# ricklisz/AnatoMask

Hardware: AMD Instinct MI355X
Metric: pretrain volumes/sec @128^3 patch mask=0.6 (higher is better)
Workload: dtype bf16; 1 GPU; STUNet-B AnatoMask step, 128^3 patch, mask_ratio 0.6, bf16 storage/MFMA + fp32 master; per_gpu_batch=16, global_batch=16, parallelism=dp1, step=teacher fwd + sampler + student fwd + loss + bwd + clip + AdamW + EMA

## Files before the change

### anatomask_amd/csrc/stream_ops.hip

```cpp
#include <mutex>
#include <type_traits>
#include "common.h"
#include "../../include/anatomask_hip.h"

namespace {

constexpr int NREP = 8;

struct Geo {
  int B, D, H, W, C;
  int vpw;
  unsigned mW, mH, mD;
  MaskView mask;
  __device__ __forceinline__ bool active(long v) const {
    if (!mask.m) return true;
    const unsigned u = (unsigned)v;
    const unsigned t1 = __umulhi(u, mW); const int w = u - t1 * W;
    const unsigned t2 = __umulhi(t1, mH); const int h = t1 - t2 * H;
    const unsigned b = __umulhi(t2, mD); const int d = t2 - b * D;
    return mask.active((int)b, d, h, w);
  }
  __device__ __forceinline__ void decode(long v, int& b, int& d, int& h, int& w) const {
    const unsigned u = (unsigned)v;
    const unsigned t1 = __umulhi(u, mW); w = u - t1 * W;
// ... 1242 lines not shown
    const double b1 = wc * S0, b2 = rs * wc * S1;
    const float gr = fin.gamma[c] * fin.rstd[c];
    fin.k0w[c] = gr * fin.w[c]; fin.k1[c] = gr * (float)(b1 / fin.n); fin.k2[c] = gr * (float)(b2 / fin.n);
    fin.dgamma[c] += (float)b2;
    fin.dbeta[c] += (float)b1;
    fin.dw[c] += (float)((double)fin.scale[c] * S1 + (double)fin.beta[c] * S0);
  }
  if (threadIdx.x == 0) atomicExch(fin.ticket, 0u);
}

template <typename T>
__global__ __launch_bounds__(256) void proj_norm_bwd_apply_kernel(const T* __restrict__ x, const float* __restrict__ drec, long nvox, int C,
                                                                  int vpw, const float* __restrict__ mean, const float* __restrict__ rstd,
                                                                  const float* __restrict__ k0w, const float* __restrict__ k1,
                                                                  const float* __restrict__ k2, T* __restrict__ dx) {
  constexpr int EPC = TT<T>::EPC;
  Walk<T> wk(C);
  if (!wk.live) return;
  float mu[EPC], c0[EPC], c1[EPC], c2[EPC];
#pragma unroll
  for (int i = 0; i < EPC; ++i) {
    const int c = wk.cl * EPC + i;
    mu[i] = mean[c]; c0[i] = k0w[c]; c1[i] = k1[c]; c2[i] = k2[c] * rstd[c];
  }
  const long v0 = (long)blockIdx.x * vpw, v1 = min(v0 + (long)vpw, nvox);
  for (long v = v0 + wk.vl; v < v1; v += wk.vpp) {
    const float d = drec[v];
    const size_t off = (size_t)v * C + wk.cl * EPC;
    float f[EPC], r[EPC];
    chunk_to_f<T>(*(const u32x4*)(x + off), f);
#pragma unroll
    for (int i = 0; i < EPC; ++i) r[i] = c0[i] * d - c1[i] - c2[i] * (f[i] - mu[i]);
    *(u32x4*)(dx + off) = f_to_chunk<T>(r);
  }
}

template <typename T>
__global__ __launch_bounds__(256) void proj_bwd_kernel(const T* __restrict__ x, const float* __restrict__ drec, long nvox, int C, int vpw,
                                                       const float* __restrict__ w, T* __restrict__ dx, float* __restrict__ dw,
                                                       float* __restrict__ db, float* __restrict__ det_ws) {
  constexpr int EPC = TT<T>::EPC;
  __shared__ float red[256 * 8];
  __shared__ float redb[4];
  Walk<T> wk(C);
  float sw[EPC], wv[EPC], sb = 0.f;
#pragma unroll
  for (int i = 0; i < EPC; ++i) { sw[i] = 0.f; wv[i] = wk.live ? w[wk.cl * EPC + i] : 0.f; }
  const long v0 = (long)blockIdx.x * vpw, v1 = min(v0 + (long)vpw, nvox);
  if (wk.live)
    for (long v = v0 + wk.vl; v < v1; v += wk.vpp) {
      const float d = drec[v];
      const size_t off = (size_t)v * C + wk.cl * EPC;
      float f[EPC], o[EPC];
      chunk_to_f<T>(*(const u32x4*)(x + off), f);
#pragma unroll
      for (int i = 0; i < EPC; ++i) { sw[i] += d * f[i]; o[i] = d * wv[i]; }
      *(u32x4*)(dx + off) = f_to_chunk<T>(o);
      if (wk.cl == 0) sb += d;
    }
#pragma unroll
  for (int i = 0; i < EPC; ++i) red[threadIdx.x * 8 + i] = sw[i];
  sb = warp_sum(sb);
  if ((threadIdx.x & 63) == 0) redb[threadIdx.x >> 6] = sb;
  __syncthreads();
  if (threadIdx.x < wk.cpv) {
    float a1[EPC];
// ... 597 lines not shown
  hipStream_t st = (hipStream_t)stream;
  const int nb = (int)((nvox + 255) / 256);
  am_by_dtype(dtype, [&](auto t) {
    using T = typename decltype(t)::type;
    AM_LAUNCH(proj_fwd_kernel<T>, dim3(nb), dim3(256), 0, st, (const T*)x, nvox, C, w, b, pre_scale, pre_shift, rec);
  });
  AM_CHECK_LAUNCH();
  return 0;
}

int am_proj_norm_bwd(int dtype, const void* x, const float* drec, long nvox, int C, const float* w, const float* gamma, const float* beta,
                     const float* mean, const float* rstd, const float* scale, double* workspace, float* coef, void* dx,
                     float* dgamma_accum, float* dbeta_accum, float* dw_accum, float* db_accum, void* stream) {
  if (!am_row_ok(dtype, C, F32_MAX_C_256)) return -1;
  if (!x || !drec || !w || !gamma || !beta || !mean || !rstd || !scale || !workspace || !coef || !dx || !dgamma_accum || !dbeta_accum ||
      !dw_accum || !db_accum || nvox <= 0) return -1;
  hipStream_t st = (hipStream_t)stream;
  ProjNormFin fin{(unsigned*)(workspace + (size_t)NREP * (C + 1)), (double)nvox, gamma, beta, rstd, scale, w,
                  coef, coef + C, coef + 2 * C, dgamma_accum, dbeta_accum, dw_accum, db_accum};
  const int vr = pick_vpw(nvox, C, dtype, true), va = pick_vpw(nvox, C, dtype, false);
  am_by_dtype(dtype, [&](auto t) {
    using T = typename decltype(t)::type;
    AM_LAUNCH(proj_norm_bwd_reduce_kernel<T>, dim3(nblk(nvox, vr)), dim3(256), 0, st, (const T*)x, drec, nvox, C, vr, mean, workspace, fin);
  });
  AM_CHECK_LAUNCH();
  am_by_dtype(dtype, [&](auto t) {
    using T = typename decltype(t)::type;
    AM_LAUNCH(proj_norm_bwd_apply_kernel<T>, dim3(nblk(nvox, va)), dim3(256), 0, st, (const T*)x, drec, nvox, C, va, mean, rstd, coef, coef + C, coef + 2 * C, (T*)dx);
  });
  AM_CHECK_LAUNCH();
  return 0;
}

int am_proj_bwd(int dtype, const void* x, const float* drec, long nvox, int C, const float* w, void* dx, float* dw_accum,
                float* db_accum, float* det_workspace, long det_workspace_floats, void* stream) {
  if (!am_row_ok(dtype, C, F32_MAX_C_256)) return -1;
  hipStream_t st = (hipStream_t)stream;
  const int vpw = pick_vpw(nvox, C, dtype, true);
  const int nb = nblk(nvox, vpw);
  if (det_workspace && det_workspace_floats < (long)nb * (C + 1)) return -6;
  am_by_dtype(dtype, [&](auto t) {
    using T = typename decltype(t)::type;
    AM_LAUNCH(proj_bwd_kernel<T>, dim3(nb), dim3(256), 0, st, (const T*)x, drec, nvox, C, vpw, w, (T*)dx, dw_accum, db_accum, det_workspace);
  });
  AM_CHECK_LAUNCH();
  if (det_workspace) {
    AM_LAUNCH(rows_fold_kernel, dim3((C + 1 + 255) / 256), dim3(256), 0, st, det_workspace, nb, C + 1, C, dw_accum, db_accum);
    AM_CHECK_LAUNCH();
  }
  return 0;
}

int am_partials_reduce(const float* partials, int rows, int C, double* sums, float* sum_accum, void* stream) {
  hipStream_t st = (hipStream_t)stream;
  if ((256 % C == 0 || C % 256 == 0) && rows >= 64) {
    const int rstep = C <= 256 ? 256 / C : 1;
    int nb = rows / (rstep * 16); nb = nb < 1 ? 1 : (nb > 256 ? 256 : nb);
    const int rpb = ((rows + nb - 1) / nb + rstep - 1) / rstep * rstep;
    nb = (rows + rpb - 1) / rpb;
    if (sums) AM_HIP(hipMemsetAsync(sums, 0, sizeof(double) * 2 * C, st));
    AM_LAUNCH(partials_reduce2_kernel, dim3(nb), dim3(256), 0, st, partials, rows, C, rpb, sums, sum_accum);
    AM_CHECK_LAUNCH();
    return 0;
  }
  AM_LAUNCH(partials_reduce_kernel, dim3(C), dim3(256), 0, st, partials, rows, C, sums, sum_accum);
  AM_CHECK_LAUNCH();
// ... 78 lines not shown
```

### anatomask_amd/engine.py

```python
from __future__ import annotations

from dataclasses import dataclass, field
from typing import Dict, List, Optional, Sequence, Tuple

import torch

from . import ops
from .ops import ACT_LRELU, ACT_NONE, ACT_RELU6, CONV_DGRAD, CONV_FWD, CONVT_DGRAD, CONVT_FWD, MaskInfo, NormStats

ENC = "sparse_encoder.sp_cnn.conv_blocks_context"
DEC = "dense_decoder.dec"


@dataclass
class Spec:
    dims: Sequence[int]
    depth: Sequence[int]
    width: int
    input_size: Tuple[int, int, int]
    in_ch: int = 1
    out_ch: int = 1
    downsample: int = 16
    n_stage: int = 5
    sync_bn: bool = False
    dec_inorm: bool = False
    enc_chs: List[int] = field(init=False)
    dec_chs: List[int] = field(init=False)
    fmap: Tuple[int, int, int] = field(init=False)

    def __post_init__(self):
        assert self.in_ch == 1 and self.out_ch == 1, "the AnatoMask recipe is single-channel CT (P/pretrain_AntoMask.py:188)"
        assert all(s % self.downsample == 0 for s in self.input_size)
        self.enc_chs = list(self.dims[:5])
        n = 4
        self.dec_chs = [self.width // 2 ** i for i in range(n + 1)]
        self.fmap = tuple(s // self.downsample for s in self.input_size)
        assert all(c % 8 == 0 for c in self.enc_chs + self.dec_chs), "channel counts must be multiples of 8"

    def stage_spatial(self, s: int) -> Tuple[int, int, int]:
        return tuple(v >> s for v in self.input_size)


class Tape:

    def __init__(self):
        self.enc: List[dict] = []
        self.dens: List[dict] = []
        self.dec: List[dict] = []
        self.last: Optional[torch.Tensor] = None
        self.counts: Dict[int, torch.Tensor] = {}
        self.recompute = False
        self.enc_in: List[Optional[torch.Tensor]] = []


def _counts(mask: MaskInfo, levels: Sequence[int]) -> Dict[int, object]:
    if mask.n_active is not None:
        return {bs: float(mask.n_active) * float((1 << bs) ** 3) for bs in levels}
    out = {}
    buf = torch.empty(len(levels), device=mask.t.device, dtype=torch.float64)
    for i, bs in enumerate(levels):
        ops.mask_count(mask, (1 << bs) ** 3, buf[i:i + 1])
        out[bs] = buf[i:i + 1]
    return out


def _set_count(st: NormStats, cnt):
    if isinstance(cnt, float):
        st.count_host, st.count_ptr = cnt, None
    else:
        st.count_ptr = cnt


def _sparse_norm(x, mask, bs, counts, gamma, beta, eps, part=None) -> NormStats:
    st = NormStats(x.shape[-1], x.device)
    _set_count(st, counts[bs])
    if part is not None:
        part.finalize(st, gamma, beta, eps)
        return st
    ops.chan_stats(x, mask, bs, st)
    ops.norm_finalize(st, gamma, beta, eps)
    return st


def _sync_world(sync: bool) -> int:
    import torch.distributed as dist
# ... 203 lines not shown
        if tape is not None and recompute:
            tape.enc_in.append(x)
        for b in range(spec.depth[s]):
            x, rec_ = _enc_block(W, pk, inp, mask, counts, sp, s, b, x, keep=tape is not None)
            if tape is not None and not recompute:
                tape.enc.append(rec_)
        feats.append(x)
    return feats


def densify_forward(spec: Spec, W, pk: PackCache, feats, mask: MaskInfo, counts, tape: Optional[Tape] = None) -> List[torch.Tensor]:
    n_dec = len(spec.dec_chs) - 1
    to_dec = []
    for i in range(n_dec):
        f = feats[4 - i]
        st = _sparse_norm(f, mask, i, counts, W[f"densify_norms.{i}.weight"], W[f"densify_norms.{i}.bias"], 1e-6)
        d = ops.norm_apply(f, st, ACT_NONE, mask, i, fill=W[f"mask_tokens.{i}"].view(-1))
        pw = f"densify_projs.{i}.weight"
        if pw in W:
            k = W[pw].shape[-1]
            pr = ops.conv3d(CONV_FWD, d, pk.get(W, pw, False, False), W[f"densify_projs.{i}.bias"], tuple(d.shape[1:4]), k, 1)
        else:
            pr = d
        to_dec.append(pr)
        if tape is not None:
            tape.dens.append({"i": i, "f": f, "st": st, "d": d, "k": W[pw].shape[-1] if pw in W else 0})
    return to_dec


HEAD_STENCIL = True


def decoder_forward(spec: Spec, W, pk: PackCache, to_dec, train: bool, tape: Optional[Tape] = None, recompute: bool = False,
                    needed_patches: Optional[MaskInfo] = None, fuse_eval: Optional[bool] = None, l2_of: Optional[tuple] = None) -> torch.Tensor:
    n_dec = len(spec.dec_chs) - 1
    if fuse_eval is None:
        fuse_eval = tape is None
    x = to_dec[0]
    head = bool(train and FUSED_HEAD and _sync_world(spec.sync_bn) <= 1 and not spec.dec_inorm)
    st_head = None
    for i in range(n_dec):
        nxt = to_dec[i + 1] if i + 1 < n_dec else None
        last = i == n_dec - 1
        o, rec_ = _dec_block(W, pk, i, x, nxt, train, fuse_eval=fuse_eval,
                             out_skip=needed_patches if (last and tape is None and not train) else None, sync=spec.sync_bn,
                             head=head and last, inorm=spec.dec_inorm,
                             stencil_tail=bool(HEAD_STENCIL and last and tape is None and not train and fuse_eval and not spec.dec_inorm))
        if rec_ is not None and rec_.get("stencil"):
            q = f"{DEC}.{i}"
            weff, beff = ops.head_fold(W[f"{q}.conv.3.weight"], rec_["st2"].scale, rec_["st2"].shift, W["dense_decoder.proj.weight"].view(-1),
                                       W["dense_decoder.proj.bias"])
            B_, D_, H_, W_ = o.shape[:4]
            patches = needed_patches
            if patches is None:
                patches = MaskInfo(torch.ones(B_, D_ // 16, H_ // 16, W_ // 16, device=o.device, dtype=torch.uint8), n_active=B_ * (D_ // 16) * (H_ // 16) * (W_ // 16))
            if l2_of is not None:
                ops.head_stencil(o, weff, beff, patches, inp=l2_of[0], l2=l2_of[1])
                return None
            rec = torch.empty(B_, D_, H_, W_, device=o.device, dtype=torch.float32)
            ops.head_stencil(o, weff, beff, patches, rec=rec)
            return rec
        if head and last:
            st_head = rec_["st2"]
        if tape is not None:
            tape.dec.append({"q": rec_["q"], "xin": x, "nxt": nxt, "head": head and last} if recompute else rec_)
        x = o
    rec = ops.proj_fwd(x, W["dense_decoder.proj.weight"].view(-1), W["dense_decoder.proj.bias"], pre=st_head)
    if tape is not None:
        tape.last = x
    return rec


def forward(spec: Spec, W: Dict[str, torch.Tensor], pk: PackCache, inp: torch.Tensor, mask: MaskInfo, train: bool,
            tape: Optional[Tape] = None, want_feats: bool = False, encoder_only: bool = False, recompute: bool = False,
            want_to_dec0: bool = False, needed_patches: Optional[MaskInfo] = None, l2_out: Optional[torch.Tensor] = None):
    counts = _counts(mask, range(5))
    if tape is not None:
        tape.counts = counts
        tape.recompute = recompute
    feats = encoder_forward(spec, W, pk, inp, mask, counts, tape, recompute)
    if encoder_only:
        return feats
    to_dec = densify_forward(spec, W, pk, feats, mask, counts, tape)
    rec = decoder_forward(spec, W, pk, to_dec, train, tape, recompute, needed_patches, l2_of=(inp, l2_out) if l2_out is not None else None)
    if want_to_dec0:
        return rec, to_dec[0]
    return (rec, feats) if want_feats else rec


FUSED_HEAD = True
_SIDE: Dict[int, "torch.cuda.Stream"] = {}
_SIDE_KEEP: Dict[int, List[torch.Tensor]] = {}
_USE_SIDE = True


def _dev_index(dev) -> int:
    return dev.index if dev.index is not None else torch.cuda.current_device()


def _side_stream(dev) -> "torch.cuda.Stream":
    i = _dev_index(dev)
    if i not in _SIDE:
        _SIDE[i] = torch.cuda.Stream(device=dev)
    return _SIDE[i]


def _on_side(dev, tensors, fn):
    if not _USE_SIDE:
        return fn()
    s2 = _side_stream(dev)
    ev = torch.cuda.Event()
    ev.record()
    s2.wait_event(ev)
    _SIDE_KEEP.setdefault(_dev_index(dev), []).extend(tensors)
    with torch.cuda.stream(s2):
        fn()


def _join_side(dev):
    i = _dev_index(dev)
    if _USE_SIDE and i in _SIDE:
        ev = torch.cuda.Event()
        ev.record(_SIDE[i])
        torch.cuda.current_stream(dev).wait_event(ev)
    _SIDE_KEEP.pop(i, None)


def _wgrad_into(pk: PackCache, G, name, mode, x, dy, k, stride, transposed=False, **masks):
    def run():
        dwp = ops.conv3d_wgrad(mode, x, dy, k, stride, f32_split=pk.f32_split, deterministic=pk.deterministic, **masks)
        ops.unpack_grad(dwp, G[name], transposed, accumulate=True)
    _on_side(x.device, (x, dy), run)


def _dec_block_backward(W, G, pk: PackCache, t: dict, g: Optional[torch.Tensor], drec: Optional[torch.Tensor], bias_sum_into: Optional[torch.Tensor]):
    q = t["q"]
    if t.get("inorm"):
        so = tuple(t["r"].shape[1:4])
        dc2 = _instance_norm_backward(g, t["c2"], t["st2"], ACT_NONE)
        dr = ops.conv3d(CONV_DGRAD, dc2, pk.get(W, f"{q}.conv.3.weight", False, True), None, so, 3, 1)
        _wgrad_into(pk, G, f"{q}.conv.3.weight", CONV_FWD, t["r"], dc2, 3, 1)
        dc1 = _instance_norm_backward(dr, t["c1"], t["st1"], ACT_RELU6)
    elif t.get("head"):
        dc2 = ops.proj_norm_bwd(t["c2"], t["st2"], drec, W["dense_decoder.proj.weight"].view(-1), W[f"{q}.conv.4.weight"],
                                W[f"{q}.conv.4.bias"], G[f"{q}.conv.4.weight"], G[f"{q}.conv.4.bias"],
                                G["dense_decoder.proj.weight"].view(-1), G["dense_decoder.proj.bias"])
    else:
        dc2 = ops.norm_backward(g, None, t["c2"], t["st2"], W[f"{q}.conv.4.weight"], ACT_NONE, None, 0,
                                G[f"{q}.conv.4.weight"], G[f"{q}.conv.4.bias"])
    if not t.get("inorm"):
        so = tuple(t["r"].shape[1:4])
        fuse = ops.FUSED_NORM_BWD_REDUCE and dc2.dtype == torch.bfloat16 and t["st1"].sync_world <= 1 and dc2.shape[-1] >= 128
        dr = ops.conv3d(CONV_DGRAD, dc2, pk.get(W, f"{q}.conv.3.weight", False, True), None, so, 3, 1,
                        norm_bwd=(t["c1"], t["st1"], ACT_RELU6) if fuse else None)
        dr, red1 = dr if fuse else (dr, None)
        _wgrad_into(pk, G, f"{q}.conv.3.weight", CONV_FWD, t["r"], dc2, 3, 1)
        dc1 = ops.norm_backward(dr, None, t["c1"], t["st1"], W[f"{q}.conv.1.weight"], ACT_RELU6, None, 0,
                                G[f"{q}.conv.1.weight"], G[f"{q}.conv.1.bias"], reduced=red1)
    du, ptu = ops.conv3d(CONV_DGRAD, dc1, pk.get(W, f"{q}.conv.0.weight", False, True), None, so, 3, 1, want_partials=True, partials_sum_only=True)
    ptu.finalize(None, sum_accum=G[f"{q}.up_sample.bias"])
    _wgrad_into(pk, G, f"{q}.conv.0.weight", CONV_FWD, t["u"], dc1, 3, 1)
    si = tuple(t["xin"].shape[1:4])
    gin = ops.conv3d(CONVT_DGRAD, du, pk.get(W, f"{q}.up_sample.weight", True, True), None, si, 4, 2, want_partials=bias_sum_into is not None)
    if bias_sum_into is not None:
        gin, ptg = gin
        ptg.finalize(None, sum_accum=bias_sum_into)
    _wgrad_into(pk, G, f"{q}.up_sample.weight", CONVT_FWD, t["xin"], du, 4, 2, transposed=True)
    return gin


def decoder_backward(spec: Spec, W, G, pk: PackCache, tape: Tape, drec: torch.Tensor, after_group=None) -> List[Optional[torch.Tensor]]:
    n_dec = len(spec.dec_chs) - 1
    fused_head = bool(tape.dec[n_dec - 1].get("head"))
    g = None
    if not fused_head:
        g = ops.proj_bwd(tape.last, drec, W["dense_decoder.proj.weight"].view(-1), G["dense_decoder.proj.weight"].view(-1),
                         G["dense_decoder.proj.bias"], deterministic=pk.deterministic)
        if after_group:
            after_group("proj")
    dproj: List[Optional[torch.Tensor]] = [None] * n_dec
    for i in reversed(range(n_dec)):
        t = tape.dec[i]
        if tape.recompute:
            _, t = _dec_block(W, pk, i, t["xin"], t["nxt"], True, update_running=False, sync=spec.sync_bn, head=bool(t.get("head")),
                              inorm=spec.dec_inorm)
            tape.dec[i] = None
        if i + 1 < n_dec:
            dproj[i + 1] = g
        need_sum = i > 0 and f"densify_projs.{i}.bias" in G
        g = _dec_block_backward(W, G, pk, t, g, drec, G[f"densify_projs.{i}.bias"] if need_sum else None)
        if t.get("head") and after_group:
            after_group("proj")
        if after_group:
            after_group(f"dec{i}")
    dproj[0] = g
    return dproj


def densify_backward(spec: Spec, W, G, pk: PackCache, mask: MaskInfo, tape: Tape, dproj) -> List[Optional[torch.Tensor]]:
    n_dec = len(spec.dec_chs) - 1
    dfeat: List[Optional[torch.Tensor]] = [None] * spec.n_stage
    for i in range(n_dec):
        t = tape.dens[i]
        dp = dproj[i]
        if t["k"]:
            pw = f"densify_projs.{i}.weight"
            dd = ops.conv3d(CONV_DGRAD, dp, pk.get(W, pw, False, True), None, tuple(dp.shape[1:4]), t["k"], 1)
            _wgrad_into(pk, G, pw, CONV_FWD, t["d"], dp, t["k"], 1)
            if i == 0:
                ops.chan_sum(dp, None, 0, G[f"densify_projs.{i}.bias"])
        else:
            dd = dp
        dfeat[4 - i] = ops.norm_backward(dd, None, t["f"], t["st"], W[f"densify_norms.{i}.weight"], ACT_NONE, mask, i,
                                         G[f"densify_norms.{i}.weight"], G[f"densify_norms.{i}.bias"],
                                         dtoken=G[f"mask_tokens.{i}"].view(-1), fill=True)
    return dfeat


def _enc_block_backward(W, G, pk: PackCache, inp: torch.Tensor, mask: MaskInfo, t: dict, gout: torch.Tensor, base: Optional[torch.Tensor],
                        free_saved: bool = False) -> Optional[torch.Tensor]:
    p, s = t["p"], t["s"]
    bs = 4 - s
    y2, a1, y1, out, x = t["y2"], t["a1"], t["y1"], t["out"], t["x"]
# ... 127 lines not shown
```

### anatomask_amd/ops.py

```python
from __future__ import annotations

from typing import Optional, Tuple

import torch

from . import hip
from .hip import ACT_LRELU, ACT_NONE, ACT_RELU6, CONV_DGRAD, CONV_FWD, CONVT_DGRAD, CONVT_FWD


def _dt(t: torch.Tensor) -> int:
    if t.dtype == torch.float32:
        return hip.DT_F32
    if t.dtype == torch.bfloat16:
        return hip.DT_BF16
    raise TypeError(f"unsupported dtype {t.dtype}")


DEFAULT_F32_SPLIT = False


def _dtc(t: torch.Tensor, f32_split: bool) -> int:
    return hip.DT_F32S if (t.dtype == torch.float32 and f32_split) else _dt(t)


# ... 466 lines not shown
    B, D, H, W, Cc = x.shape
    mp, fd, fh, fw = _mk(mask)
    hip.lib().chan_sum(_dt(x), x.data_ptr(), B, D, H, W, Cc, mp, bshift, fd, fh, fw, out_accum.data_ptr(), _stream())


def add(a: torch.Tensor, b: torch.Tensor, out: Optional[torch.Tensor] = None) -> torch.Tensor:
    if out is None:
        out = torch.empty_like(a)
    hip.lib().add(_dt(a), a.data_ptr(), b.data_ptr(), out.data_ptr(), a.numel(), _stream())
    return out


def proj_fwd(x: torch.Tensor, w: torch.Tensor, b: torch.Tensor, pre: Optional["NormStats"] = None) -> torch.Tensor:
    B, D, H, W, Cc = x.shape
    rec = torch.empty(B, D, H, W, device=x.device, dtype=torch.float32)
    hip.lib().proj_fwd(_dt(x), x.data_ptr(), B * D * H * W, Cc, w.data_ptr(), b.data_ptr(), _p(pre.scale) if pre else None,
                       _p(pre.shift) if pre else None, rec.data_ptr(), _stream())
    return rec


def proj_norm_bwd(x: torch.Tensor, st: "NormStats", drec: torch.Tensor, w: torch.Tensor, gamma: torch.Tensor, beta: torch.Tensor,
                  dgamma: torch.Tensor, dbeta: torch.Tensor, dw_accum: torch.Tensor, db_accum: torch.Tensor) -> torch.Tensor:
    B, D, H, W, Cc = x.shape
    assert st.sync_world <= 1
    dx = torch.empty_like(x)
    ws_b, _ = _bwd_workspaces(x.device, Cc)
    coef = torch.empty(3, Cc, device=x.device, dtype=torch.float32)
    hip.lib().proj_norm_bwd(_dt(x), x.data_ptr(), drec.data_ptr(), B * D * H * W, Cc, w.data_ptr(), gamma.data_ptr(), beta.data_ptr(),
                            st.mean.data_ptr(), st.rstd.data_ptr(), st.scale.data_ptr(), ws_b.data_ptr(), coef.data_ptr(), dx.data_ptr(),
                            dgamma.data_ptr(), dbeta.data_ptr(), dw_accum.data_ptr(), db_accum.data_ptr(), _stream())
    return dx


def proj_bwd(x: torch.Tensor, drec: torch.Tensor, w: torch.Tensor, dw_accum: torch.Tensor, db_accum: torch.Tensor,
             deterministic: Optional[bool] = None) -> torch.Tensor:
    B, D, H, W, Cc = x.shape
    dx = torch.empty_like(x)
    ws = _det_workspace(x.device, 4096 * (Cc + 1) // 8) if _det(deterministic) else None
    hip.lib().proj_bwd(_dt(x), x.data_ptr(), drec.data_ptr(), B * D * H * W, Cc, w.data_ptr(), dx.data_ptr(), dw_accum.data_ptr(),
                       db_accum.data_ptr(), _p(ws), ws.numel() if ws is not None else 0, _stream())
    return dx


def head_stencil_supported(x: torch.Tensor) -> bool:
    B, D, H, W, C = x.shape
    ok = hip.lib()._lib.am_head_stencil_supported(_dt(x), C) == 1
    return bool(ok and D % 16 == 0 and H % 16 == 0 and W % 16 == 0 and max(B, D // 16, H // 16, W // 16) <= 255)


def head_fold(w2: torch.Tensor, scale: torch.Tensor, shift: torch.Tensor, wproj: torch.Tensor, bproj: torch.Tensor):
    cmid, cin = w2.shape[0], w2.shape[1]
    assert tuple(w2.shape[2:]) == (3, 3, 3) and w2.is_contiguous() and wproj.numel() == cmid
    weff = torch.empty(27, cin, device=w2.device, dtype=torch.float32)
    beff = torch.empty(1, device=w2.device, dtype=torch.float32)
    hip.lib().head_fold(w2.data_ptr(), cmid, cin, scale.data_ptr(), shift.data_ptr(), wproj.data_ptr(), bproj.data_ptr(), weff.data_ptr(),
                        beff.data_ptr(), _stream())
    return weff, beff


def head_stencil(r: torch.Tensor, weff: torch.Tensor, beff: torch.Tensor, patches: MaskInfo, rec: Optional[torch.Tensor] = None,
                 inp: Optional[torch.Tensor] = None, l2: Optional[torch.Tensor] = None):
    B, D, H, W, C = r.shape
    lst, n = patches.active_list()
    assert lst is not None and (patches.fd, patches.fh, patches.fw) == (D // 16, H // 16, W // 16) and r.is_contiguous()
    assert rec is None or (rec.dtype == torch.float32 and tuple(rec.shape) == (B, D, H, W) and rec.is_contiguous())
    assert l2 is None or (inp is not None and l2.dtype == torch.float32 and l2.numel() == B * patches.fd * patches.fh * patches.fw)
# ... 133 lines not shown
```

### anatomask_amd/trainer.py

```python
from __future__ import annotations

from typing import Dict, Optional

import torch
import torch.distributed as dist

from . import engine, ops
from .modules import ModelEma, SparK, ema_decay_for_epoch


class _Range:
    __slots__ = ("on",)

    def __init__(self, on: bool, name: str):
        self.on = on
        if on:
            torch.cuda.nvtx.range_push(name)

    def __enter__(self):
        return self

    def __exit__(self, *exc):
        if self.on:
            torch.cuda.nvtx.range_pop()
# ... 213 lines not shown
    def step(self, inp_bchwd: torch.Tensor, epoch: int = 0, mask1: Optional[torch.Tensor] = None,
             keys: Optional[torch.Tensor] = None, lr: Optional[float] = None, ema_decay: Optional[float] = None):
        m, t = self.model, self.teacher.ema
        spec = m.spec
        x = inp_bchwd[:, 0].float().contiguous()
        B = x.shape[0]
        L = spec.fmap[0] * spec.fmap[1] * spec.fmap[2]
        dev = x.device
        if mask1 is None:
            k1 = torch.rand(B, L, device=dev, generator=self.gen)
            m1 = ops.mask_sampler(torch.zeros(B, L, device=dev), k1, m.len_keep, 0)
        else:
            m1 = mask1.reshape(B, L).to(device=dev, dtype=torch.uint8).contiguous()
        mi1 = ops.MaskInfo(m1.view(B, *spec.fmap), n_active=B * m.len_keep if mask1 is None else None)
        tr_ = self.trace_ranges
        if self.self_distill:
            with _Range(tr_, "anatomask.teacher_forward"):
                need = ops.MaskInfo((1 - m1).view(B, *spec.fmap), n_active=B * (L - m.len_keep) if mask1 is None else None) if spec.input_size[0] // spec.fmap[0] == 16 else None
                recon = torch.zeros(B, L, device=dev) if need is not None else None
                rec1 = engine.forward(spec, t._W, t._pack, x, mi1, train=False, needed_patches=need, l2_out=recon)
                if rec1 is not None:
                    recon, _, _, _ = ops.patch_loss_fwd(x, rec1, mi1, normalized=False, want_loss=False)
                del rec1
            with _Range(tr_, "anatomask.mask_sampler"):
                ll = m.len_loss_for(L, m.len_keep, epoch, self.total_epochs - 1, self.guide)
                if keys is None:
                    keys = torch.rand(B, L, device=dev, generator=self.gen)
                mk = ops.mask_sampler(recon, keys.to(dev).float().contiguous(), m.len_keep, ll)
                mi = ops.MaskInfo(mk.view(B, *spec.fmap), n_active=B * m.len_keep)
        else:
            recon, mk, mi = None, m1, mi1
        self._snap_b.copy_(m._bflat); self._snap_i.copy_(m._iflat)
        tape = engine.Tape()
        with _Range(tr_, "anatomask.student_forward"):
            rec = engine.forward(spec, m._W, m._pack, x, mi, train=True, tape=tape, recompute=m.recompute)
            l2m, pm, pr, info = ops.patch_loss_fwd(x, rec, mi, normalized=True)
            drec = ops.patch_loss_bwd(x, rec, mi, pm, pr, info, None)
        with _Range(tr_, "anatomask.backward"):
            m._gflat.zero_()
            if self.distributed and not self._capturing:
                self._exchange_begin()
            engine.backward(spec, m._W, m._G, m._pack, x, mi, tape, drec, self._after_group if self.distributed else None, join_before_hook=False)
            del tape
        with _Range(tr_, "anatomask.exchange_wait"):
            self._finish_exchange()
        rng_opt = _Range(tr_, "anatomask.optimizer_ema")
        n = m._live_end
        decay = self.teacher.decay if ema_decay is None else ema_decay
        ops.sumsq(m._gflat[:n], self.sumsq)
        dyn = None
        if self._capturing:
            dyn = self._dyn_dev
        else:
            self.step_count += 1
        ops.adamw_ema(m._flat, m._gflat, self.m, self.v, t._flat if self.self_distill else None, n, self.lr if lr is None else lr,
                      self.betas, self.eps, self.wd, max(self.step_count, 1), self.sumsq, self.clip, decay, self.gnorm,
                      grad_scale=self.grad_scale, dyn=dyn, guard=self.guard)
        ops.guard_restore(m._bflat, self._snap_b, self.guard)
        ops.guard_restore(m._iflat, self._snap_i, self.guard)
        if not self.self_distill:
            m.weights_changed()
            rng_opt.__exit__()
            return {"loss": info[0:1], "grad_norm": self.gnorm, "mask": mk, "recon_loss": None, "rec_loss": l2m}
        if m._flat.numel() > n:
            ops.ema(t._flat[n:], m._flat[n:], decay, self.guard)
        ops.ema(t._bflat, m._bflat, decay, self.guard)
        if m._n_ibuf:
            ops.ema_i64(t._iflat[:m._n_ibuf], m._iflat[:m._n_ibuf], decay, self.guard)
        m.weights_changed(); t.weights_changed()
        rng_opt.__exit__()
        return {"loss": info[0:1], "grad_norm": self.gnorm, "mask": mk, "recon_loss": recon, "rec_loss": l2m}

# ... 64 lines not shown
```

### include/anatomask_hip.h

```cpp
#ifndef ANATOMASK_HIP_H
#define ANATOMASK_HIP_H
#include <stdint.h>
#ifdef __cplusplus
extern "C" {
#endif

#define AM_DT_F32 0
#define AM_DT_BF16 1
#define AM_DT_F32S 2

#define AM_CONV_PARTIALS_SUM_ONLY 2
#define AM_CONV_FWD 0
#define AM_CONV_DGRAD 1
#define AM_CONVT_FWD 2
#define AM_CONVT_DGRAD 3

#define AM_DXREP 64
#define AM_NREP 8

#define AM_ACT_NONE 0
#define AM_ACT_LRELU 1
#define AM_ACT_RELU6 2

int am_version(void);
// ... 90 lines not shown
                       const float* pre_scale, const float* pre_shift ,
                       const int32_t* active_list, int n_active,
                       const double* count_ptr, double count_host, const float* gamma, float* k0, float* k1, float* k2,
                       float* dgamma_accum, float* dbeta_accum, float* dtoken_accum, float* dbeta2_accum
                       ,
                       void* stream);
int am_norm_bwd_finalize(const double* bsum, const double* count_ptr, double count_host, int C, const float* gamma,
                         const float* rstd, float* k0, float* k1, float* k2, float* dgamma_accum, float* dbeta_accum,
                         float* dtoken_accum, float* dbeta2_accum , void* stream);
int am_norm_bwd_apply(int dtype, const void* dout, const void* out, const void* x, int B, int D, int H, int W, int C,
                      const uint8_t* mask, int bshift, int fd, int fh, int fw, const float* mean, const float* rstd,
                      const float* k0, const float* k1, const float* k2, int act, void* dx, void* dres,
                      float* dxsum_accum ,
                      double* dxsum_scratch ,
                      const float* pre_scale, const float* pre_shift ,
                      const int32_t* active_list, int n_active,
                      int scratch_is_zero_workspace , void* stream);
int am_chan_sum(int dtype, const void* x, int B, int D, int H, int W, int C, const uint8_t* mask, int bshift, int fd, int fh,
                int fw, float* out_accum, void* stream);
int am_add(int dtype, const void* a, const void* b, void* y, long n_elems, void* stream);

int am_head_fold(const float* w2, int cmid, int cin, const float* scale, const float* shift, const float* wproj, const float* bproj,
                 float* weff, float* beff, void* stream);
int am_head_stencil(int dtype, const void* r, int B, int D, int H, int W, int C, const float* weff, const float* beff,
                    const int32_t* patch_list, int n_patches, float* rec , const float* inp ,
                    float* l2 , void* stream);
int am_head_stencil_supported(int dtype, int C);

int am_proj_fwd(int dtype, const void* x, long nvox, int C, const float* w, const float* b,
                const float* pre_scale, const float* pre_shift , float* rec, void* stream);
int am_proj_norm_bwd(int dtype, const void* x, const float* drec, long nvox, int C, const float* w, const float* gamma, const float* beta,
                     const float* mean, const float* rstd, const float* scale, double* workspace, float* coef, void* dx,
                     float* dgamma_accum, float* dbeta_accum, float* dw_accum, float* db_accum, void* stream);
int am_proj_bwd(int dtype, const void* x, const float* drec, long nvox, int C, const float* w, void* dx, float* dw_accum,
                float* db_accum, float* det_workspace, long det_workspace_floats , void* stream);

int am_patch_loss_fwd(const float* inp, const float* rec, const uint8_t* active, int B, int D, int H, int W, int normalized,
                      float* l2m, float* pmean, float* prstd, float* lossinfo, void* stream);
int am_patch_loss_bwd(const float* inp, const float* rec, const uint8_t* active, int B, int D, int H, int W, const float* pmean,
                      const float* prstd, const float* lossinfo, const float* gout, float* drec, void* stream);

int am_mask_sampler(const float* loss, const float* keys, int B, int L, int len_keep, int len_loss, uint8_t* mask, void* stream);

int am_sumsq(const float* g, long n, double* out, void* stream);
int am_adamw_ema(float* p, const float* g, float* m, float* v, float* ema , long n, double lr, double beta1,
                 double beta2, double eps, double weight_decay, int step, const double* sumsq ,
                 double max_norm, double ema_decay, double grad_scale ,
                 float* gnorm_out,
                 const float* dyn_scalars ,
                 int* guard ,
                 void* stream);
int am_ema(float* ema, const float* p, long n, double decay, const int* guard , void* stream);
int am_ema_i64(long* ema, const long* p, int n, double decay, const int* guard, void* stream);
int am_guard_restore(void* dst, const void* snapshot, long nbytes, const int* guard, void* stream);

int am_spline_prefilter(float* vol, int D, int H, int W, void* stream);
int am_resample_affine(const float* src, int Ds, int Hs, int Ws, float* dst, int D, int H, int W, const float* affine_host12, int order,
                       float cval, void* stream);


#define AM_LAYER_REP 64
int am_voxel_norm_fwd(int dtype, int kind, const void* x, void* y, int B, int D, int H, int W, int C, int groups, const float* gamma,
                      const float* beta, float eps, const uint8_t* mask, int bshift, const int32_t* active_list, int n_active, void* stream);
int am_voxel_norm_bwd(int dtype, int kind, const void* x, const void* dy, void* dx, int B, int D, int H, int W, int C, int groups,
                      const float* gamma, float eps, float* dgamma_accum, float* dbeta_accum, const uint8_t* mask, int bshift,
                      const int32_t* active_list, int n_active, void* stream);
// ... 45 lines not shown
```

Measured before the change: 140.1 volumes/s.

## Fuse decoder head projection with patch-normalized loss and its backward

Adds head_loss_fwd/bwd kernels that compute the 1x1 projection of the final decoder features, per-patch input normalization, masked L2 loss, and the proj-norm backward reductions in one pass per 16^3 patch. The full-resolution rec and drec fp32 volumes are never materialized, and the separate proj_fwd, patch_loss_fwd/bwd and proj_norm_bwd reduce kernels are removed. The backward recomputes rec from x instead of reading it. Gradient zeroing moves before the forward because the fused forward now accumulates into gradient buffers. The risk is extra per-voxel reduction work inside the kernels and a last-workgroup finalization step.

Result: no change. 141.0 volumes/s, median of 6 (+0.6%).

```diff
diff --git a/anatomask_amd/csrc/stream_ops.hip b/anatomask_amd/csrc/stream_ops.hip
--- a/anatomask_amd/csrc/stream_ops.hip
+++ b/anatomask_amd/csrc/stream_ops.hip
@@ -1298,6 +1298,225 @@
 #pragma unroll
     for (int i = 0; i < EPC; ++i) r[i] = c0[i] * d - c1[i] - c2[i] * (f[i] - mu[i]);
     *(u32x4*)(dx + off) = f_to_chunk<T>(r);
+  }
+}
+
+template <bool FAST>
+__device__ __forceinline__ float voxel_sum(float p, int cpv, int vl, bool live, float* part) {
+  if constexpr (FAST) {
+    for (int o = cpv >> 1; o > 0; o >>= 1) p += __shfl_xor(p, o, 64);
+    return p;
+  }
+  __syncthreads();
+  part[threadIdx.x] = p;
+  __syncthreads();
+  float s = 0.f;
+  if (live)
+    for (int c = 0; c < cpv; ++c) s += part[vl * cpv + c];
+  return s;
+}
+
+__device__ __forceinline__ float block_sum256(float v, float* sh) {
+  v = warp_sum(v);
+  __syncthreads();
+  if ((threadIdx.x & 63) == 0) sh[threadIdx.x >> 6] = v;
+  __syncthreads();
+  return sh[0] + sh[1] + sh[2] + sh[3];
+}
+
+struct HeadLossGeo {
+  const float* inp; const uint8_t* active;
+  int D, H, W, fd, fh, fw, C;
+  const float *w, *b, *psc, *psh, *mean;
+};
+
+template <typename T, bool FAST>
+__global__ __launch_bounds__(256) void head_loss_fwd_kernel(const T* __restrict__ x, HeadLossGeo a, float* __restrict__ l2m,
+                                                            float* __restrict__ pmean, float* __restrict__ prstd,
+                                                            float* __restrict__ lossinfo, double* __restrict__ acc, ProjNormFin fin) {
+  constexpr int EPC = TT<T>::EPC;
+  __shared__ float xin[4096];
+  __shared__ float red[256 * 8];
+  __shared__ float part[256];
+  __shared__ float sh[4];
+  __shared__ double s0sh;
+  __shared__ float ksh;
+  const int C = a.C, AW = C + 2;
+  if (a.active[blockIdx.x]) {
+    if (threadIdx.x == 0) { l2m[blockIdx.x] = 0.f; pmean[blockIdx.x] = 0.f; prstd[blockIdx.x] = 1.f; }
+  } else {
+    const int L = a.fd * a.fh * a.fw;
+    const int b = blockIdx.x / L, l = blockIdx.x % L;
+    const int pw = l % a.fw, ph = (l / a.fw) % a.fh, pd = l / (a.fw * a.fh);
+    const size_t pbase = (((size_t)b * a.D + pd * 16) * a.H + ph * 16) * a.W + pw * 16;
+    float mean, rstd;
+    {
+      const int z = threadIdx.x >> 4, y = threadIdx.x & 15;
+      const size_t base = pbase + ((size_t)z * a.H + y) * a.W;
+      float xi[16];
+#pragma unroll
+      for (int q = 0; q < 4; ++q) {
+        const f32x4 t = *(const f32x4*)(a.inp + base + 4 * q);
+#pragma unroll
+        for (int i = 0; i < 4; ++i) xi[4 * q + i] = t[i];
+      }
+      float s = 0.f;
+#pragma unroll
+      for (int i = 0; i < 16; ++i) s += xi[i];
+      mean = block_sum256(s, sh) * (1.f / 4096.f);
+      float s2 = 0.f;
+#pragma unroll
+      for (int i = 0; i < 16; ++i) { const float d = xi[i] - mean; s2 += d * d; }
+      const float var = block_sum256(s2, sh) * (1.f / 4095.f);
+      rstd = 1.f / sqrtf(var + 1e-6f);
+#pragma unroll
+      for (int i = 0; i < 16; ++i) xin[threadIdx.x * 16 + i] = xi[i];
+    }
+    __syncthreads();
+    Walk<T> wk(C);
+    float aw[EPC], mu[EPC], s1[EPC], p0 = 0.f, e = 0.f, sb = 0.f;
+#pragma unroll
+    for (int i = 0; i < EPC; ++i) {
+      const int c = wk.cl * EPC + i;
+      s1[i] = 0.f;
+      aw[i] = wk.live ? a.w[c] * a.psc[c] : 0.f; mu[i] = wk.live ? a.mean[c] : 0.f;
+      if (wk.live) p0 += a.w[c] * a.psh[c];
+    }
+    const float bias = a.b[0];
+    const int npass = (4096 + wk.vpp - 1) / wk.vpp;
+    constexpr int U = FAST ? 4 : 1;
+    for (int it = 0; it < npass; it += U) {
+      float f[U][EPC];
+      bool ok[U];
+#pragma unroll
+      for (int u = 0; u < U; ++u) {
+        const int j = (it + u) * wk.vpp + wk.vl;
+        ok[u] = FAST || (wk.live && j < 4096);
+        if (ok[u]) {
+          const size_t v = pbase + ((size_t)(j >> 8) * a.H + ((j >> 4) & 15)) * a.W + (j & 15);
+          chunk_to_f<T>(*(const u32x4*)(x + v * C + wk.cl * EPC), f[u]);
+        }
+      }
+#pragma unroll
+      for (int u = 0; u < U; ++u) {
+        const int j = (it + u) * wk.vpp + wk.vl;
+        float p = p0;
+        if (ok[u])
+#pragma unroll
+          for (int i = 0; i < EPC; ++i) p += f[u][i] * aw[i];
+        const float rec = bias + voxel_sum<FAST>(p, wk.cpv, wk.vl, wk.live, part);
+        if (ok[u]) {
+          const float q = rec - (xin[j] - mean) * rstd;
+#pragma unroll
+          for (int i = 0; i < EPC; ++i) s1[i] += q * (f[u][i] - mu[i]);
+          if (wk.cl == 0) { e += q * q; sb += q; }
+        }
+      }
+    }
+#pragma unroll
+    for (int i = 0; i < EPC; ++i) red[threadIdx.x * 8 + i] = s1[i];
+    e = block_sum256(e, sh) * (1.f / 4096.f);
+    sb = block_sum256(sb, sh);
+    double* ar = acc + (size_t)(blockIdx.x % NREP) * AW;
+    if (threadIdx.x < wk.cpv) {
+      double a1[EPC];
+#pragma unroll
+      for (int i = 0; i < EPC; ++i) a1[i] = 0.0;
+      for (int vl = 0; vl < wk.vpp; ++vl)
+#pragma unroll
+        for (int i = 0; i < EPC; ++i) a1[i] += red[(vl * wk.cpv + threadIdx.x) * 8 + i];
+#pragma unroll
+      for (int i = 0; i < EPC; ++i) atomicAdd(&ar[threadIdx.x * EPC + i], a1[i]);
+    }
+    if (threadIdx.x == 0) {
+      l2m[blockIdx.x] = e; pmean[blockIdx.x] = mean; prstd[blockIdx.x] = rstd;
+      atomicAdd(&ar[C], (double)sb); atomicAdd(&ar[C + 1], (double)e);
+    }
+  }
+  if (!last_workgroup(fin.ticket)) return;
+  float cnt = 0.f;
+  for (int i = threadIdx.x; i < (int)gridDim.x; i += 256) cnt += a.active[i] ? 0.f : 1.f;
+  cnt = block_sum256(cnt, sh);
+  if (threadIdx.x == 0) {
+    double t = 0.0, ls = 0.0;
+    for (int r = 0; r < NREP; ++r) {
+      t += __longlong_as_double(atomicExch((unsigned long long*)&acc[(size_t)r * AW + C], 0ull));
+      ls += __longlong_as_double(atomicExch((unsigned long long*)&acc[(size_t)r * AW + C + 1], 0ull));
+    }
+    const float lossv = (float)ls / (cnt + 1e-8f), inv = 1.f / (cnt + 1e-8f);
+    lossinfo[0] = lossv; lossinfo[1] = inv;
+    const float k = lossv - lossv == 0.f ? inv * (2.f / 4096.f) : __builtin_nanf("");
+    ksh = k;
+    s0sh = t * (double)k;
+    fin.db[0] += (float)s0sh;
+  }
+  __syncthreads();
+  const double S0 = s0sh, kd = (double)ksh;
+  for (int c = threadIdx.x; c < C; c += blockDim.x) {
+    double S1 = 0.0;
+    for (int r = 0; r < NREP; ++r) S1 += __longlong_as_double(atomicExch((unsigned long long*)&acc[(size_t)r * AW + c], 0ull));
+    S1 *= kd;
+    const double wc = fin.w[c], rs = fin.rstd[c];
+    const double b1 = wc * S0, b2 = rs * wc * S1;
+    const float gr = fin.gamma[c] * fin.rstd[c];
+    fin.k0w[c] = gr * fin.w[c]; fin.k1[c] = gr * (float)(b1 / fin.n); fin.k2[c] = gr * (float)(b2 / fin.n);
+    fin.dgamma[c] += (float)b2;
+    fin.dbeta[c] += (float)b1;
+    fin.dw[c] += (float)((double)fin.scale[c] * S1 + (double)fin.beta[c] * S0);
+  }
+  if (threadIdx.x == 0) atomicExch(fin.ticket, 0u);
+}
+
+struct HeadLossBwd {
+  const float *pmean, *prstd, *lossinfo, *rstd, *k0w, *k1, *k2;
+  long nvox; int vpw, W16;
+  unsigned mW16, mH, mD;
+};
+
+template <typename T, bool FAST>
+__global__ __launch_bounds__(256) void head_loss_bwd_kernel(const T* __restrict__ x, HeadLossGeo a, HeadLossBwd g, T* __restrict__ dx) {
+  constexpr int EPC = TT<T>::EPC;
+  __shared__ float part[256];
+  const int C = a.C;
+  Walk<T> wk(C);
+  float aw[EPC], mu[EPC], c0[EPC], c1[EPC], c2[EPC], p0 = 0.f;
+#pragma unroll
+  for (int i = 0; i < EPC; ++i) {
+    const int c = wk.cl * EPC + i;
+    aw[i] = wk.live ? a.w[c] * a.psc[c] : 0.f; mu[i] = wk.live ? a.mean[c] : 0.f;
+    if (wk.live) p0 += a.w[c] * a.psh[c];
+    c0[i] = wk.live ? g.k0w[c] : 0.f; c1[i] = wk.live ? g.k1[c] : 0.f; c2[i] = wk.live ? g.k2[c] * g.rstd[c] : 0.f;
+  }
+  const float bias = a.b[0];
+  const float lossv = g.lossinfo[0];
+  const float k = lossv - lossv == 0.f ? g.lossinfo[1] * (2.f / 4096.f) : __builtin_nanf("");
+  const long v0 = (long)blockIdx.x * g.vpw, v1 = min(v0 + (long)g.vpw, g.nvox);
+  const int npass = (int)((v1 - v0 + wk.vpp - 1) / wk.vpp);
+  for (int it = 0; it < npass; ++it) {
+    const long v = v0 + (long)it * wk.vpp + wk.vl;
+    const bool ok = FAST || (wk.live && v < v1);
+    const size_t off = (size_t)v * C + wk.cl * EPC;
+    float f[EPC], p = p0;
+    int pi = 0;
+    if (ok) {
+      chunk_to_f<T>(*(const u32x4*)(x + off), f);
+      const unsigned s = (unsigned)(v >> 4);
+      const unsigned t1 = g.W16 == 1 ? s : __umulhi(s, g.mW16); const int pw = s - t1 * g.W16;
+      const unsigned t2 = __umulhi(t1, g.mH); const int h = t1 - t2 * a.H;
+      const unsigned bb = __umulhi(t2, g.mD); const int d = t2 - bb * a.D;
+      pi = (((int)bb * a.fd + (d >> 4)) * a.fh + (h >> 4)) * a.fw + pw;
+#pragma unroll
+      for (int i = 0; i < EPC; ++i) p += f[i] * aw[i];
+    }
+    const float rec = bias + voxel_sum<FAST>(p, wk.cpv, wk.vl, wk.live, part);
+    if (ok) {
+      float d = 0.f;
+      if (!a.active[pi]) d = k * (rec - (a.inp[v] - g.pmean[pi]) * g.prstd[pi]);
+      float r[EPC];
+#pragma unroll
+      for (int i = 0; i < EPC; ++i) r[i] = c0[i] * d - c1[i] - c2[i] * (f[i] - mu[i]);
+      *(u32x4*)(dx + off) = f_to_chunk<T>(r);
+    }
   }
 }
 
@@ -1961,6 +2180,60 @@
   return 0;
 }
 
+static bool head_loss_geo_ok(int dtype, int B, int D, int H, int W, int C) {
+  if (!am_row_ok(dtype, C, F32_MAX_C_256) || B <= 0 || D <= 0 || H <= 0 || W <= 0 || D % 16 || H % 16 || W % 16) return false;
+  const unsigned long long runs = (unsigned long long)B * D * H * (W / 16);
+  int m = W / 16 > H ? W / 16 : H; if (D > m) m = D;
+  return runs * (unsigned long long)m < 0xffffffffull && (unsigned long long)B * (D / 16) * (H / 16) * (W / 16) <= 0x7fffffffull;
+}
+static bool head_loss_fast(int dtype, int C) {
+  const int cpv = C / (dtype == AM_DT_BF16 ? 8 : 4);
+  return cpv <= 64 && (cpv & (cpv - 1)) == 0;
+}
+
+int am_head_loss_fwd(int dtype, const void* x, const float* inp, const uint8_t* active, int B, int D, int H, int W, int C, const float* w,
+                     const float* b, const float* gamma, const float* beta, const float* mean, const float* rstd, const float* scale,
+                     const float* shift, double* workspace, float* coef, float* l2m, float* pmean, float* prstd, float* lossinfo,
+                     float* dgamma_accum, float* dbeta_accum, float* dw_accum, float* db_accum, void* stream) {
+  if (!head_loss_geo_ok(dtype, B, D, H, W, C)) return -1;
+  if (!x || !inp || !active || !w || !b || !gamma || !beta || !mean || !rstd || !scale || !shift || !workspace || !coef || !l2m || !pmean ||
+      !prstd || !lossinfo || !dgamma_accum || !dbeta_accum || !dw_accum || !db_accum) return -1;
+  hipStream_t st = (hipStream_t)stream;
+  const int fd = D / 16, fh = H / 16, fw = W / 16;
+  HeadLossGeo a{inp, active, D, H, W, fd, fh, fw, C, w, b, scale, shift, mean};
+  ProjNormFin fin{(unsigned*)(workspace + (size_t)NREP * (C + 2)), (double)B * D * H * W, gamma, beta, rstd, scale, w,
+                  coef, coef + C, coef + 2 * C, dgamma_accum, dbeta_accum, dw_accum, db_accum};
+  const bool fast = head_loss_fast(dtype, C);
+  am_by_dtype(dtype, [&](auto t) {
+    using T = typename decltype(t)::type;
+    if (fast) AM_LAUNCH((head_loss_fwd_kernel<T, true>), dim3(B * fd * fh * fw), dim3(256), 0, st, (const T*)x, a, l2m, pmean, prstd, lossinfo, workspace, fin);
+    else AM_LAUNCH((head_loss_fwd_kernel<T, false>), dim3(B * fd * fh * fw), dim3(256), 0, st, (const T*)x, a, l2m, pmean, prstd, lossinfo, workspace, fin);
+  });
+  AM_CHECK_LAUNCH();
+  return 0;
+}
+
+int am_head_loss_bwd(int dtype, const void* x, const float* inp, const uint8_t* active, int B, int D, int H, int W, int C, const float* w,
+                     const float* b, const float* mean, const float* rstd, const float* scale, const float* shift, const float* pmean,
+                     const float* prstd, const float* lossinfo, const float* coef, void* dx, void* stream) {
+  if (!head_loss_geo_ok(dtype, B, D, H, W, C)) return -1;
+  if (!x || !inp || !active || !w || !b || !mean || !rstd || !scale || !shift || !pmean || !prstd || !lossinfo || !coef || !dx) return -1;
+  hipStream_t st = (hipStream_t)stream;
+  const long nvox = (long)B * D * H * W;
+  HeadLossGeo a{inp, active, D, H, W, D / 16, H / 16, W / 16, C, w, b, scale, shift, mean};
+  HeadLossBwd g{pmean, prstd, lossinfo, rstd, coef, coef + C, coef + 2 * C, nvox, pick_vpw(nvox, C, dtype, false), W / 16,
+                (unsigned)(0x100000000ull / (unsigned)(W / 16)) + 1, (unsigned)(0x100000000ull / (unsigned)H) + 1,
+                (unsigned)(0x100000000ull / (unsigned)D) + 1};
+  const bool fast = head_loss_fast(dtype, C);
+  am_by_dtype(dtype, [&](auto t) {
+    using T = typename decltype(t)::type;
+    if (fast) AM_LAUNCH((head_loss_bwd_kernel<T, true>), dim3(nblk(nvox, g.vpw)), dim3(256), 0, st, (const T*)x, a, g, (T*)dx);
+    else AM_LAUNCH((head_loss_bwd_kernel<T, false>), dim3(nblk(nvox, g.vpw)), dim3(256), 0, st, (const T*)x, a, g, (T*)dx);
+  });
+  AM_CHECK_LAUNCH();
+  return 0;
+}
+
 int am_proj_bwd(int dtype, const void* x, const float* drec, long nvox, int C, const float* w, void* dx, float* dw_accum,
                 float* db_accum, float* det_workspace, long det_workspace_floats, void* stream) {
   if (!am_row_ok(dtype, C, F32_MAX_C_256)) return -1;
diff --git a/anatomask_amd/engine.py b/anatomask_amd/engine.py
--- a/anatomask_amd/engine.py
+++ b/anatomask_amd/engine.py
@@ -51,6 +51,7 @@
         self.counts: Dict[int, torch.Tensor] = {}
         self.recompute = False
         self.enc_in: List[Optional[torch.Tensor]] = []
+        self.head_loss: Optional[dict] = None
 
 
 def _counts(mask: MaskInfo, levels: Sequence[int]) -> Dict[int, object]:
@@ -320,7 +321,8 @@
 
 
 def decoder_forward(spec: Spec, W, pk: PackCache, to_dec, train: bool, tape: Optional[Tape] = None, recompute: bool = False,
-                    needed_patches: Optional[MaskInfo] = None, fuse_eval: Optional[bool] = None, l2_of: Optional[tuple] = None) -> torch.Tensor:
+                    needed_patches: Optional[MaskInfo] = None, fuse_eval: Optional[bool] = None, l2_of: Optional[tuple] = None,
+                    head_loss: Optional[tuple] = None) -> torch.Tensor:
     n_dec = len(spec.dec_chs) - 1
     if fuse_eval is None:
         fuse_eval = tape is None
@@ -353,6 +355,15 @@
         if tape is not None:
             tape.dec.append({"q": rec_["q"], "xin": x, "nxt": nxt, "head": head and last} if recompute else rec_)
         x = o
+    if head_loss is not None and tape is not None and st_head is not None and _head_loss_on(x, head_loss[1]):
+        inp, mi, G = head_loss
+        q = f"{DEC}.{n_dec - 1}"
+        l2m, pm, pr, info, coef = ops.head_loss_fwd(x, st_head, inp, mi, W["dense_decoder.proj.weight"].view(-1), W["dense_decoder.proj.bias"],
+                                                    W[f"{q}.conv.4.weight"], W[f"{q}.conv.4.bias"], G[f"{q}.conv.4.weight"], G[f"{q}.conv.4.bias"],
+                                                    G["dense_decoder.proj.weight"].view(-1), G["dense_decoder.proj.bias"])
+        tape.head_loss = {"inp": inp, "mask": mi, "l2m": l2m, "pm": pm, "pr": pr, "info": info, "coef": coef}
+        tape.last = x
+        return None
     rec = ops.proj_fwd(x, W["dense_decoder.proj.weight"].view(-1), W["dense_decoder.proj.bias"], pre=st_head)
     if tape is not None:
         tape.last = x
@@ -361,7 +372,8 @@
 
 def forward(spec: Spec, W: Dict[str, torch.Tensor], pk: PackCache, inp: torch.Tensor, mask: MaskInfo, train: bool,
             tape: Optional[Tape] = None, want_feats: bool = False, encoder_only: bool = False, recompute: bool = False,
-            want_to_dec0: bool = False, needed_patches: Optional[MaskInfo] = None, l2_out: Optional[torch.Tensor] = None):
+            want_to_dec0: bool = False, needed_patches: Optional[MaskInfo] = None, l2_out: Optional[torch.Tensor] = None,
+            head_loss_into: Optional[Dict[str, torch.Tensor]] = None):
     counts = _counts(mask, range(5))
     if tape is not None:
         tape.counts = counts
@@ -370,13 +382,19 @@
     if encoder_only:
         return feats
     to_dec = densify_forward(spec, W, pk, feats, mask, counts, tape)
-    rec = decoder_forward(spec, W, pk, to_dec, train, tape, recompute, needed_patches, l2_of=(inp, l2_out) if l2_out is not None else None)
+    rec = decoder_forward(spec, W, pk, to_dec, train, tape, recompute, needed_patches, l2_of=(inp, l2_out) if l2_out is not None else None,
+                          head_loss=(inp, mask, head_loss_into) if head_loss_into is not None else None)
     if want_to_dec0:
         return rec, to_dec[0]
     return (rec, feats) if want_feats else rec
 
 
 FUSED_HEAD = True
+FUSED_HEAD_LOSS = True
+
+
+def _head_loss_on(c2: torch.Tensor, mask: MaskInfo) -> bool:
+    return bool(FUSED_HEAD_LOSS and tuple(c2.shape[1:4]) == (16 * mask.fd, 16 * mask.fh, 16 * mask.fw) and ops.head_loss_supported(c2))
 _SIDE: Dict[int, "torch.cuda.Stream"] = {}
 _SIDE_KEEP: Dict[int, List[torch.Tensor]] = {}
 _USE_SIDE = True
@@ -421,7 +439,8 @@
     _on_side(x.device, (x, dy), run)
 
 
-def _dec_block_backward(W, G, pk: PackCache, t: dict, g: Optional[torch.Tensor], drec: Optional[torch.Tensor], bias_sum_into: Optional[torch.Tensor]):
+def _dec_block_backward(W, G, pk: PackCache, t: dict, g: Optional[torch.Tensor], drec: Optional[torch.Tensor], bias_sum_into: Optional[torch.Tensor],
+                        head_loss: Optional[dict] = None):
     q = t["q"]
     if t.get("inorm"):
         so = tuple(t["r"].shape[1:4])
@@ -429,6 +448,10 @@
         dr = ops.conv3d(CONV_DGRAD, dc2, pk.get(W, f"{q}.conv.3.weight", False, True), None, so, 3, 1)
         _wgrad_into(pk, G, f"{q}.conv.3.weight", CONV_FWD, t["r"], dc2, 3, 1)
         dc1 = _instance_norm_backward(dr, t["c1"], t["st1"], ACT_RELU6)
+    elif t.get("head") and head_loss is not None:
+        hl = head_loss
+        dc2 = ops.head_loss_bwd(t["c2"], t["st2"], hl["inp"], hl["mask"], W["dense_decoder.proj.weight"].view(-1), W["dense_decoder.proj.bias"],
+                                hl["pm"], hl["pr"], hl["info"], hl["coef"])
     elif t.get("head"):
         dc2 = ops.proj_norm_bwd(t["c2"], t["st2"], drec, W["dense_decoder.proj.weight"].view(-1), W[f"{q}.conv.4.weight"],
                                 W[f"{q}.conv.4.bias"], G[f"{q}.conv.4.weight"], G[f"{q}.conv.4.bias"],
@@ -476,7 +499,8 @@
         if i + 1 < n_dec:
             dproj[i + 1] = g
         need_sum = i > 0 and f"densify_projs.{i}.bias" in G
-        g = _dec_block_backward(W, G, pk, t, g, drec, G[f"densify_projs.{i}.bias"] if need_sum else None)
+        g = _dec_block_backward(W, G, pk, t, g, drec, G[f"densify_projs.{i}.bias"] if need_sum else None,
+                                head_loss=tape.head_loss if i == n_dec - 1 else None)
         if t.get("head") and after_group:
             after_group("proj")
         if after_group:
diff --git a/anatomask_amd/ops.py b/anatomask_amd/ops.py
--- a/anatomask_amd/ops.py
+++ b/anatomask_amd/ops.py
@@ -522,6 +522,39 @@
     return dx
 
 
+def head_loss_supported(x: torch.Tensor) -> bool:
+    B, D, H, W, Cc = x.shape
+    if D % 16 or H % 16 or W % 16 or Cc % 8 or Cc > (2048 if x.dtype == torch.bfloat16 else 1024):
+        return False
+    return B * D * H * (W // 16) * max(W // 16, H, D) < 0xffffffff
+
+
+def head_loss_fwd(x: torch.Tensor, st: "NormStats", inp: torch.Tensor, mask: MaskInfo, w: torch.Tensor, b: torch.Tensor, gamma: torch.Tensor,
+                  beta: torch.Tensor, dgamma: torch.Tensor, dbeta: torch.Tensor, dw_accum: torch.Tensor, db_accum: torch.Tensor):
+    B, D, H, W, Cc = x.shape
+    assert st.sync_world <= 1 and (mask.fd, mask.fh, mask.fw) == (D // 16, H // 16, W // 16) and tuple(inp.shape) == (B, D, H, W)
+    L = mask.fd * mask.fh * mask.fw
+    l2m, pm, pr = (torch.empty(B, L, device=x.device, dtype=torch.float32) for _ in range(3))
+    info = torch.empty(2, device=x.device, dtype=torch.float32)
+    coef = torch.empty(3, Cc, device=x.device, dtype=torch.float32)
+    ws_b, _ = _bwd_workspaces(x.device, Cc)
+    hip.lib().head_loss_fwd(_dt(x), x.data_ptr(), inp.data_ptr(), mask.t.data_ptr(), B, D, H, W, Cc, w.data_ptr(), b.data_ptr(),
+                            gamma.data_ptr(), beta.data_ptr(), st.mean.data_ptr(), st.rstd.data_ptr(), st.scale.data_ptr(),
+                            st.shift.data_ptr(), ws_b.data_ptr(), coef.data_ptr(), l2m.data_ptr(), pm.data_ptr(), pr.data_ptr(),
+                            info.data_ptr(), dgamma.data_ptr(), dbeta.data_ptr(), dw_accum.data_ptr(), db_accum.data_ptr(), _stream())
+    return l2m, pm, pr, info, coef
+
+
+def head_loss_bwd(x: torch.Tensor, st: "NormStats", inp: torch.Tensor, mask: MaskInfo, w: torch.Tensor, b: torch.Tensor, pm: torch.Tensor,
+                  pr: torch.Tensor, info: torch.Tensor, coef: torch.Tensor) -> torch.Tensor:
+    B, D, H, W, Cc = x.shape
+    dx = torch.empty_like(x)
+    hip.lib().head_loss_bwd(_dt(x), x.data_ptr(), inp.data_ptr(), mask.t.data_ptr(), B, D, H, W, Cc, w.data_ptr(), b.data_ptr(),
+                            st.mean.data_ptr(), st.rstd.data_ptr(), st.scale.data_ptr(), st.shift.data_ptr(), pm.data_ptr(), pr.data_ptr(),
+                            info.data_ptr(), coef.data_ptr(), dx.data_ptr(), _stream())
+    return dx
+
+
 def proj_bwd(x: torch.Tensor, drec: torch.Tensor, w: torch.Tensor, dw_accum: torch.Tensor, db_accum: torch.Tensor,
              deterministic: Optional[bool] = None) -> torch.Tensor:
     B, D, H, W, Cc = x.shape
diff --git a/anatomask_amd/trainer.py b/anatomask_amd/trainer.py
--- a/anatomask_amd/trainer.py
+++ b/anatomask_amd/trainer.py
@@ -269,12 +269,16 @@
             recon, mk, mi = None, m1, mi1
         self._snap_b.copy_(m._bflat); self._snap_i.copy_(m._iflat)
         tape = engine.Tape()
+        m._gflat.zero_()
         with _Range(tr_, "anatomask.student_forward"):
-            rec = engine.forward(spec, m._W, m._pack, x, mi, train=True, tape=tape, recompute=m.recompute)
-            l2m, pm, pr, info = ops.patch_loss_fwd(x, rec, mi, normalized=True)
-            drec = ops.patch_loss_bwd(x, rec, mi, pm, pr, info, None)
+            rec = engine.forward(spec, m._W, m._pack, x, mi, train=True, tape=tape, recompute=m.recompute, head_loss_into=m._G)
+            if rec is None:
+                l2m, info, drec = tape.head_loss["l2m"], tape.head_loss["info"], None
+            else:
+                l2m, pm, pr, info = ops.patch_loss_fwd(x, rec, mi, normalized=True)
+                drec = ops.patch_loss_bwd(x, rec, mi, pm, pr, info, None)
+            del rec
         with _Range(tr_, "anatomask.backward"):
-            m._gflat.zero_()
             if self.distributed and not self._capturing:
                 self._exchange_begin()
             engine.backward(spec, m._W, m._G, m._pack, x, mi, tape, drec, self._after_group if self.distributed else None, join_before_hook=False)
diff --git a/include/anatomask_hip.h b/include/anatomask_hip.h
--- a/include/anatomask_hip.h
+++ b/include/anatomask_hip.h
@@ -146,6 +146,13 @@
 int am_proj_norm_bwd(int dtype, const void* x, const float* drec, long nvox, int C, const float* w, const float* gamma, const float* beta,
                      const float* mean, const float* rstd, const float* scale, double* workspace, float* coef, void* dx,
                      float* dgamma_accum, float* dbeta_accum, float* dw_accum, float* db_accum, void* stream);
+int am_head_loss_fwd(int dtype, const void* x, const float* inp, const uint8_t* active, int B, int D, int H, int W, int C, const float* w,
+                     const float* b, const float* gamma, const float* beta, const float* mean, const float* rstd, const float* scale,
+                     const float* shift, double* workspace, float* coef, float* l2m, float* pmean, float* prstd, float* lossinfo,
+                     float* dgamma_accum, float* dbeta_accum, float* dw_accum, float* db_accum, void* stream);
+int am_head_loss_bwd(int dtype, const void* x, const float* inp, const uint8_t* active, int B, int D, int H, int W, int C, const float* w,
+                     const float* b, const float* mean, const float* rstd, const float* scale, const float* shift, const float* pmean,
+                     const float* prstd, const float* lossinfo, const float* coef, void* dx, void* stream);
 int am_proj_bwd(int dtype, const void* x, const float* drec, long nvox, int C, const float* w, void* dx, float* dw_accum,
                 float* db_accum, float* det_workspace, long det_workspace_floats , void* stream);
 
```
